# African-Robotics-Unit/AcinoSet

Hardware: AMD Instinct MI355X
Metric: FTE frames/sec (residual+Jac+LM step), 6-cam x 20-joint (higher is better)
Workload: dtype f64

## Files before the change

acinoset_amd/_lib.py:

```python
import ctypes as C
import os
import subprocess

_HERE = os.path.dirname(os.path.abspath(__file__))
_CSRC = os.path.join(_HERE, "csrc")
SO_PATH = os.path.join(_HERE, "libacinoset_hip.so")
BUILD_ID_SOURCE = "camera_kernels.hip"
SOURCES = ["camera_kernels.hip", "fte_assemble.hip", "bcr.hip", "seplevel.hip", "chunk.hip", "fte_cov.hip", "fte_calib.hip", "fte_reproj.hip", "fte_api.hip", "sba.hip", "sba_cov.hip", "ekf.hip", "ekf_cov.hip", "skel_fte.hip", "skel_cov.hip", "skel_cov_rates.hip", "skel_sample.hip", "skel_calib.hip", "skel_reproj.hip"]
HEADERS = ["common.hpp", "fte_kernels.hpp", "bcr.hpp", "bcr_dev.hpp", "seplevel.hpp", "chunk.hpp", "fte_cov.hpp", "fte_cov_dev.hpp", "fte_calib.hpp", "fte_reproj.hpp", "trio80.hpp", "dense80.hpp", "cheetah_fk.hpp",
           "pinhole.hpp", "ekf_dev.hpp", "sba_dev.hpp", "sba_host.hpp", "skel_dev.hpp", "skel_host.hpp", "skel_factor.hpp", "fte_assemble_body.inc", "ekf_forward_body.inc", "skel_assemble_body.inc",
           os.path.join("..", "..", "include", "acinoset_hip.h")]

ABI_VERSION = 3
N_ACTIVE = 25
N_STATES = 45
N_MARKERS = 20
CAM_STRIDE = 24
PINHOLE_STRIDE = 32
BS = 80
SEP_DOUBLES = 2 * BS * BS + BS


class FteParams(C.Structure):
    _fields_ = [("n_frames", C.c_int32), ("n_cams", C.c_int32), ("n_global", C.c_int64), ("n_offset", C.c_int64),
# ... 160 lines not shown
    "acino_sba_solve_sharded": (_I, [C.POINTER(SbaParams), _P, _P, _P, _P, _P, _P, _P, _P, _Z, _P, _P, C.POINTER(SbaInfo),
                                     REDUCE_FN, _P, _P]),
    "acino_sizeof_sba_cov_info": (_Z, []),
    "acino_sba_covariance_workspace_bytes": (_Z, [_I, _L, _L]),
    "acino_sba_covariance": (_I, [C.POINTER(SbaParams), _P, _P, _P, _P, _P, _P, _P, _I, _I, _I, _P, _I, _P, _Z, _P, _P, _P,
                                  C.POINTER(SbaCovInfo), _P]),
    "acino_sizeof_ekf_params": (_Z, []),
    "acino_ekf_workspace_bytes": (_Z, [_L, _I]),
    "acino_ekf_run": (_I, [C.POINTER(EkfParams), _P, _P, _P, _P, _Z, _P, _P, _P, _P]),
    "acino_ekf_run_pinhole": (_I, [C.POINTER(EkfParams), _P, _P, _P, _P, _Z, _P, _P, _P, _P]),
    "acino_ekf_smoothed_covariance": (_I, [C.POINTER(EkfParams), _P, _Z, _P, _P]),
    "acino_ekf_marker_covariance": (_I, [C.POINTER(EkfParams), _P, _P, _P, _P, _P, _P]),
    "acino_skeleton_fk": (_I, [_P, _L, _I, _I, C.POINTER(SkelOp), _I, _P, _P]),
    "acino_sizeof_skel_fte_params": (_Z, []),
    "acino_sizeof_skel_fte_info": (_Z, []),
    "acino_skel_fte_workspace_bytes": (_Z, [C.POINTER(SkelFteParams)]),
    "acino_skel_fte_workspace_bytes_batch": (_Z, [C.POINTER(SkelFteParams), _I]),
    "acino_skel_fte_solve": (_I, [C.POINTER(SkelFteParams), C.POINTER(SkelOp), C.POINTER(C.c_int32), _P, _P, _P, _P, _P, _P, _P,
                                  _P, _Z, C.POINTER(SkelFteInfo), _P]),
    "acino_skel_fte_solve_batch": (_I, [C.POINTER(SkelFteParams), _I, C.POINTER(SkelOp), C.POINTER(C.c_int32), _P, _P, _P, _P, _P,
                                        _P, _P, _P, _Z, C.POINTER(SkelFteInfo), _P]),
    "acino_skel_fte_solve_pinhole": (_I, [C.POINTER(SkelFteParams), C.POINTER(SkelOp), C.POINTER(C.c_int32), _P, _P, _P, _P, _P, _P,
                                          _P, _P, _Z, C.POINTER(SkelFteInfo), _P]),
    "acino_skel_fte_solve_batch_pinhole": (_I, [C.POINTER(SkelFteParams), _I, C.POINTER(SkelOp), C.POINTER(C.c_int32), _P, _P, _P,
                                                _P, _P, _P, _P, _P, _Z, C.POINTER(SkelFteInfo), _P]),
    "acino_skel_fte_covariance_workspace_bytes": (_Z, [C.POINTER(SkelFteParams), _I]),
    "acino_skel_fte_covariance": (_I, [C.POINTER(SkelFteParams), _I, _I, C.POINTER(SkelOp), C.POINTER(C.c_int32), _P, _P, _P, _P, _P,
                                       _P, _P, _P, _P, C.POINTER(C.c_int32), _P, _Z, _P]),
    "acino_skel_fte_sample_workspace_bytes": (_Z, [C.POINTER(SkelFteParams), _I, _L]),
    "acino_skel_fte_sample": (_I, [C.POINTER(SkelFteParams), _I, _I, C.POINTER(SkelOp), C.POINTER(C.c_int32), _P, _P, _P, _P, _P,
                                   _P, _L, _P, _P, _P, C.POINTER(C.c_int32), _P, _Z, _P]),
    "acino_skel_fte_observability_workspace_bytes": (_Z, [C.POINTER(SkelFteParams), _I]),
    "acino_skel_fte_observability": (_I, [C.POINTER(SkelFteParams), _I, _I, C.POINTER(SkelOp), C.POINTER(C.c_int32), _P, _P, _P, _P,
                                          _P, _P, _P, _P, _P, _P, _Z, _P]),
    "acino_skel_fte_covariance_pinned_workspace_bytes": (_Z, [C.POINTER(SkelFteParams), _I, _I]),
    "acino_skel_fte_covariance_pinned": (_I, [C.POINTER(SkelFteParams), _I, _I, C.POINTER(SkelOp), C.POINTER(C.c_int32), _P, _P, _P,
                                              _P, _P, _P, _P, _P, _P, C.POINTER(C.c_int32), _P, _Z, _P, _I, _P]),
    "acino_skel_fte_covariance_rates_workspace_bytes": (_Z, [C.POINTER(SkelFteParams), _I, _I]),
    "acino_skel_fte_covariance_rates": (_I, [C.POINTER(SkelFteParams), _I, _I, C.POINTER(SkelOp), C.POINTER(C.c_int32), _P, _P, _P,
                                             _P, _P, _P, _P, _P, _P, _P, _P, _P, _P, C.POINTER(C.c_int32), _P, _Z, _P, _I, _P]),
    "acino_skel_fte_sample_pinned_workspace_bytes": (_Z, [C.POINTER(SkelFteParams), _I, _L, _I]),
    "acino_skel_fte_sample_pinned": (_I, [C.POINTER(SkelFteParams), _I, _I, C.POINTER(SkelOp), C.POINTER(C.c_int32), _P, _P, _P, _P,
                                          _P, _P, _L, _P, _P, _P, C.POINTER(C.c_int32), _P, _Z, _P, _I, _P]),
    "acino_skel_fte_calibration_workspace_bytes": (_Z, [C.POINTER(SkelFteParams), _I, _I]),
    "acino_skel_fte_calibration_sensitivity": (_I, [C.POINTER(SkelFteParams), _I, _I, C.POINTER(SkelOp), C.POINTER(C.c_int32), _P, _P,
                                                    _P, _P, _P, _P, _P, _P, _P, _P, _P, C.POINTER(C.c_int32), _P, _Z, _P, _I, _P]),
    "acino_skel_fte_reprojection": (_I, [C.POINTER(SkelFteParams), _I, _I, C.POINTER(SkelOp), C.POINTER(C.c_int32), _P, _P, _P, _P,
                                         _P, _D, _P, _P, _P, _P, _P, _P]),
    "acino_skel_fte_reprojection_weights": (_I, [C.POINTER(SkelFteParams), _I, _I, C.POINTER(SkelOp), C.POINTER(C.c_int32), _P, _P, _P,
                                                 _P, _P, _D, _P, _P, _P, _P, _P, _P, _P]),
    "acino_selftest_mfma": (_I, [_P, _P, _I, _P, _P]),
    "acino_debug_poison_lds": (_I, [_I, _I, _P]),
    "acino_debug_level_split": (_I, [_I, _P]),
}

_lib = None


def source_hash():
    import hashlib
    h = hashlib.sha256()
    for rel in sorted(SOURCES + HEADERS):
        path = os.path.join(_CSRC, rel)
        h.update(os.path.basename(rel).encode())
        with open(path, "rb") as f:
            h.update(f.read())
    return h.hexdigest()[:16]


def built_id():
    if not os.path.exists(SO_PATH):
        return None
    with open(SO_PATH, "rb") as f:
        blob = f.read()
    i = blob.find(b"ACINO_BUILD_ID=")
    if i < 0:
        return None
    return blob[i + 15:i + 31].decode("ascii", "replace")


def _needs_build():
    return built_id() != source_hash()


def build(force=False, verbose=False):
    if not force and not _needs_build():
        return SO_PATH
    import hashlib
    from concurrent.futures import ThreadPoolExecutor
    hipcc = os.environ.get("HIPCC", "/opt/rocm/bin/hipcc")
    if not os.path.exists(hipcc):
        hipcc = "hipcc"
    sid = source_hash()
    hdr = hashlib.sha256()
    for rel in sorted(HEADERS):
        with open(os.path.join(_CSRC, rel), "rb") as f:
            hdr.update(f.read())
    objdir = os.path.join(_CSRC, "_obj")
    os.makedirs(objdir, exist_ok=True)
    flags = ["--offload-arch=gfx950", "-O3", "-std=c++17", "-fPIC", "-DNDEBUG"]
    jobs = []
    for src in SOURCES:
        with open(os.path.join(_CSRC, src), "rb") as f:
            key = hashlib.sha256(hdr.digest() + f.read() + " ".join(flags).encode()).hexdigest()[:16]
        extra = [f'-DACINO_BUILD_ID="{sid}"'] if src == BUILD_ID_SOURCE else []
        if extra:
# ... 96 lines not shown
```

acinoset_amd/csrc/bcr_dev.hpp:

```cpp
#pragma once
#include "bcr.hpp"
#include "dense80.hpp"

namespace acino {

__device__ __forceinline__ int tri_i(int t) { return (t >= 1) + (t >= 3) + (t >= 6) + (t >= 10); }
__device__ __forceinline__ int tri_j(int t) {
  const int i = tri_i(t);
  return t - (i * (i + 1)) / 2;
}

constexpr int LOWER_ITEMS = 1920;
__device__ __forceinline__ void lower_item(int idx, int& row, int& col) {
  const int ib = (idx >= 128) + (idx >= 384) + (idx >= 768) + (idx >= 1280);
  const int rem = idx - 64 * ib * (ib + 1), w = 8 * (ib + 1);
  row = 16 * ib + rem / w;
  col = 2 * (rem % w);
}

struct NodeFetch {
  double hv[8];
  double xv, gv, lam;
  bool row_live;
};
// ... 88 lines not shown
  return build_finish(Dm, bv, f, K, t, tid, K.q_w, K.lo, K.hi);
}

template <int NTH = 256>
static __device__ void publish_gmax(double gmax, double* red, double* gn_part, int node, int tid) {
  for (int off = 32; off > 0; off >>= 1) gmax = fmax(gmax, __shfl_down(gmax, off, 64));
  if ((tid & 63) == 0) red[tid >> 6] = gmax;
  __syncthreads();
  if (tid == 0) {
    double v = red[0];
#pragma unroll
    for (int w = 1; w < NTH / 64; ++w) v = fmax(v, red[w]);
    gn_part[node] = v;
  }
}

template <int NTH, class QW>
static __device__ __forceinline__ void fill_coupling_coef_q(double* coefL, double* coefR, const FteConst& K, int node_i,
                                                            int tid, QW qw) {
  const int loc_i = 3 * (node_i - K.pin_left);
  const int64_t f_i = K.n_offset + (int64_t)loc_i;
  for (int e = tid; e < 2 * 9 * NP; e += NTH) {
    const int side = e / (9 * NP), q = e % (9 * NP), pair = q / NP, p = q % NP, ii = pair / 3, jj = pair % 3;
    if (side == 0 ? !coefL : !coefR) continue;
    double v = 0.0;
    if (ii <= jj) {
      const int k = 3 + ii - jj;
      const int hi = side == 0 ? loc_i + ii : loc_i + 3 + ii;
      if (hi < K.n_frames)
        v = 2.0 * qw(p) * (side == 0 ? band_coef_clip(f_i - 3 + jj, k, K.n_global, K.clip_len)
                                             : band_coef_clip(f_i + jj, k, K.n_global, K.clip_len));
    }
    if (side == 0) coefL[q] = v;
    else coefR[q] = v;
  }
}
template <int NTH = 256>
static __device__ __forceinline__ void fill_coupling_coef(double* coefL, double* coefR, const FteConst& K, int node_i, int tid) {
  fill_coupling_coef_q<NTH>(coefL, coefR, K, node_i, tid, [&](int p) { return K.q_w[p]; });
}
template <int NTH = 256>
static __device__ __forceinline__ void fill_coupling_coef(double* coefL, double* coefR, const FteConst& K, int node_i, int tid,
                                                          const double* qw) {
  fill_coupling_coef_q<NTH>(coefL, coefR, K, node_i, tid, [&](int p) { return qw[p]; });
}

static __device__ __forceinline__ bool coupling_tables_uniform(const FteConst& K, int first, int last) {
  if (K.clip_len > 0) return false;
  const int64_t lo = K.n_offset + 3 * (int64_t)(first - K.pin_left) - 3;
  const int64_t hi = K.n_offset + 3 * (int64_t)(last - K.pin_left) + 5;
  return lo >= 3 && hi + 3 <= K.n_global - 4 && 3 * (last - K.pin_left) + 5 < K.n_frames;
}

static __device__ __forceinline__ bool right_table_is_interior(const FteConst& K, int node) {
  const int loc = 3 * (node - K.pin_left);
  const int64_t f = K.n_offset + (int64_t)loc;
  const int64_t len = K.clip_len > 0 ? K.clip_len : K.n_global;
  const int64_t r = K.clip_len > 0 ? f % K.clip_len : f;
  return f >= 0 && r <= len - 6 && f + 5 < K.n_global && loc + 5 < K.n_frames;
}
template <int NTH, class QW>
static __device__ __forceinline__ void right_table_interior(double* coefR, int tid, QW qw) {
  for (int q = tid; q < 9 * NP; q += NTH) {
    const int pair = q / NP, p = q % NP, ii = pair / 3, jj = pair % 3;
    coefR[q] = ii <= jj ? 2.0 * qw(p) * (jj == ii ? -1.0 : (jj - ii == 1 ? 6.0 : -15.0)) : 0.0;
  }
}

__device__ __forceinline__ double* ybuf(const BcrChain& ch) { return ch.Y ? ch.Y : ch.b; }

template <int NTH>
__device__ __forceinline__ void load_node_sum(double* Lm, double* yv, const BcrChain& ch, int i, int fl, int tid) {
  constexpr int NQ = (LOWER_ITEMS + NTH - 1) / NTH;
  const size_t MB = (size_t)BS * BS;
  const double* Dg = ch.D + i * MB;
  const bool hal = ch.AL0 != nullptr, hsl = (fl & 1) != 0, hsr = (fl & 2) != 0;
  const double* Ag = hal ? ch.AL0 + i * MB : Dg;
  const double* Lg = hsl ? ch.SL + i * MB : Dg;
  const double* Rg = hsr ? ch.SR + i * MB : Dg;
  double2 dv[NQ], av[NQ], lv[NQ], rv[NQ];
#pragma unroll
  for (int k = 0; k < NQ; ++k) {
    const int idx = tid + NTH * k;
    if (idx < LOWER_ITEMS) {
      int rr, cc;
      lower_item(idx, rr, cc);
      dv[k] = *reinterpret_cast<const double2*>(Dg + rr * BS + cc);
      av[k] = *reinterpret_cast<const double2*>(Ag + rr * BS + cc);
      lv[k] = *reinterpret_cast<const double2*>(Lg + rr * BS + cc);
      rv[k] = *reinterpret_cast<const double2*>(Rg + rr * BS + cc);
    }
  }
  double bb = 0.0, ab = 0.0, lb = 0.0, rb = 0.0;
  if (tid < BS) {
    bb = ch.b[(size_t)i * BS + tid];
    const int c = tid < 3 * NP ? tid : 0;
    ab = Ag[(size_t)(BS - 1) * BS + c];
    lb = Lg[(size_t)(BS - 1) * BS + c];
    rb = Rg[(size_t)(BS - 1) * BS + c];
  }
#pragma unroll
  for (int k = 0; k < NQ; ++k) {
    const int idx = tid + NTH * k;
    if (idx < LOWER_ITEMS) {
      int rr, cc;
      lower_item(idx, rr, cc);
      const bool in0 = rr < 3 * NP && cc < 3 * NP, in1 = rr < 3 * NP && cc + 1 < 3 * NP;
      double x = dv[k].x, y = dv[k].y;
      x += (hal && in0) ? av[k].x : 0.0;
      y += (hal && in1) ? av[k].y : 0.0;
      x += (hsl && in0) ? lv[k].x : 0.0;
      y += (hsl && in1) ? lv[k].y : 0.0;
// ... 19 lines not shown
```

acinoset_amd/csrc/chunk.hip:

```cpp
#include "chunk.hpp"

#include <algorithm>
#include <cstdlib>
#include <type_traits>

#include "bcr_dev.hpp"
#include "trio80.hpp"

namespace acino {

void ChunkPlan::build(int nodes_total, int chunk_nodes, bool pin_l, bool pin_r) {
  n_nodes = nodes_total;
  m = n_chunks = n_sep = 0;
  node0 = pin_l ? 1 : 0;
  pin_right = pin_r ? 1 : 0;
  const int nodes = nodes_total - node0;
  if (chunk_nodes < 0 || nodes < 1) return;
  int mm = chunk_nodes;
  if (mm == 0) {
    mm = (nodes + 255) / 256;
    mm = std::max(4, std::min(mm, 512));
  }
  mm = std::max(2, mm);
  m = mm;
// ... 119 lines not shown
__device__ __forceinline__ void gram_fetch(const double* X, int li, int lk, double (&a)[GramTile<T>::ns], double (&b)[GramTile<T>::ns]) {
  const double* pa = X + (GramTile<T>::ib * 16 + li) * LD + GramTile<T>::ib * 16 + lk;
  const double* pb = X + (GramTile<T>::jb * 16 + li) * LD + GramTile<T>::ib * 16 + lk;
#pragma unroll
  for (int s = 0; s < GramTile<T>::ns; ++s) {
    a[s] = pa[4 * s];
    b[s] = pb[4 * s];
  }
}
template <int T>
__device__ __forceinline__ void gram_tile(double* Xg, int li, int lk, const double (&a)[GramTile<T>::ns], const double (&b)[GramTile<T>::ns]) {
  constexpr int ib = GramTile<T>::ib, jb = GramTile<T>::jb;
  d4 g = {0, 0, 0, 0};
#pragma unroll
  for (int s = 0; s < GramTile<T>::ns; ++s) g = mfma(a[s], b[s], g);
#pragma unroll
  for (int rr = 0; rr < 4; ++rr) {
    Xg[(ib * 16 + lk + 4 * rr) * LD + jb * 16 + li] = g[rr];
    if (ib != jb) Xg[(jb * 16 + li) * LD + ib * 16 + lk + 4 * rr] = g[rr];
  }
}
template <int T0, int... REST>
__device__ __forceinline__ void gram_chain(const double* Xf, double* Xg, int li, int lk, const double (&a)[GramTile<T0>::ns],
                                           const double (&b)[GramTile<T0>::ns]) {
  if constexpr (sizeof...(REST) > 0) {
    constexpr int rest[] = {REST...};
    double an[GramTile<rest[0]>::ns], bn[GramTile<rest[0]>::ns];
    gram_fetch<rest[0]>(Xf, li, lk, an, bn);
    __builtin_amdgcn_sched_barrier(0);
    gram_tile<T0>(Xg, li, lk, a, b);
    __builtin_amdgcn_sched_barrier(0);
    gram_chain<REST...>(Xf, Xg, li, lk, an, bn);
  } else {
    gram_tile<T0>(Xg, li, lk, a, b);
  }
}
template <int T0, int... REST>
__device__ __forceinline__ void gram_fixed(const double* Xf, double* Xg, int* done, int li, int lk, int lane) {
  double a[GramTile<T0>::ns], b[GramTile<T0>::ns];
  gram_fetch<T0>(Xf, li, lk, a, b);
  gram_chain<T0, REST...>(Xf, Xg, li, lk, a, b);
  asm volatile("" ::: "memory");
  if (lane == 0) __hip_atomic_fetch_add(done, 1 + (int)sizeof...(REST), __ATOMIC_RELAXED, __HIP_MEMORY_SCOPE_WORKGROUP);
  asm volatile("" ::: "memory");
}

struct SpikeArgs {
  const double* Xg;
  double* Y;
  double* Ag;
  const double* cRk;
  const double* bvn;
  double* zk;
  int *c_gfdone, *c_fready, *c_bv, *tdone;
  int *g_open, *g_done;
  const double* Xf;
  int k, n_s;
  bool hasL, has_next;
  long long* stamps;
};
template <int ROLE>
__device__ __forceinline__ void spike_node(const SpikeArgs& A, int& tsb, int ln) {
  constexpr bool two = ROLE == 5;
  constexpr int j0 = ROLE == 4 ? 1 : (ROLE == 5 ? 2 : (ROLE == 6 ? 3 : 4));
  constexpr int NA = ROLE == 4 ? 3 : (ROLE == 5 ? 2 : (ROLE == 6 ? 5 : 4));
  const int li = ln & 15, lk = ln >> 4;
  double* const Y = A.Y;
  auto stamp = [&](int i) { if (A.stamps && ln == 0) A.stamps[i] = (long long)wall_clock64(); };
  AlTiles<NA> al;
  AlTiles<1> al0;
  al.Ag = A.Ag;
  al.j = j0;
  if (ROLE == 4) { al.as[0] = 1; al.as[1] = 0; al.as[2 % NA] = 2; }
  if (ROLE == 5) { al.as[0] = 2; al.as[1] = 0; }
  if (ROLE == 6) { al.as[0] = 3; al.as[1] = 0; al.as[2 % NA] = 1; al.as[3 % NA] = 2; al.as[4 % NA] = 4; }
  if (ROLE == 7) { al.as[0] = 4; al.as[1] = 0; al.as[2 % NA] = 1; al.as[3 % NA] = 2; }
  al0.Ag = A.Ag;
  al0.j = 0;
  al0.as[0] = 0;
  if (A.hasL) {
    al.fetch(li, lk);
    if (two) al0.fetch(li, lk);
  }
  if (ROLE >= 6) {
    double* const Xg = const_cast<double*>(A.Xg);
    lds_wait(A.g_open, A.k + 1);
    if (ROLE == 6) gram_fixed<2, 13>(A.Xf, Xg, A.g_done, li, lk, ln);
    else if (A.hasL) gram_fixed<5, 9, 14>(A.Xf, Xg, A.g_done, li, lk, ln);
    else gram_fixed<2, 5, 9, 13, 14>(A.Xf, Xg, A.g_done, li, lk, ln);
  }
  lds_wait(A.g_done, 15 * (A.k + 1));
  stamp(16 + 4 * (ROLE - 4));
  d4 T0[NT], T1[NT];
  {
    double bF[NT][4];
    const double* yb = Y + lk * LD + j0 * 16 + li;
#pragma unroll
    for (int kb = 0; kb < NT; ++kb)
#pragma unroll
      for (int s = 0; s < 4; ++s) bF[kb][s] = (4 * kb + s < SP_STEPS) ? yb[(kb * 16 + 4 * s) * LD] : 0.0;
    spike_gf(A.Xg, bF, T0, li, lk);
  }
  if (two) {
    double bF[NT][4];
    const double* yb = Y + lk * LD + li;
#pragma unroll
// ... 18 lines not shown
  }
  (void)tsb;
#pragma unroll
  for (int ib = 0; ib < NT; ++ib) tile_store(Y, ib, j0, T0[ib], li, lk);
  if (two) {
#pragma unroll
    for (int ib = 0; ib < NT; ++ib) tile_store(Y, ib, 0, T1[ib], li, lk);
  }
  if (ROLE == 7) {
    A.zk[ln] = Y[ln * LD + (BS - 1)];
    if (ln < 16) A.zk[64 + ln] = Y[(64 + ln) * LD + (BS - 1)];
  }
  if (A.has_next) {
    lds_wait(A.c_bv, A.k + 1);
    const double* const cRk = A.cRk;
    const double* const bvn = A.bvn;
    const int p = ln % NP, cg = ln / NP;
#pragma unroll
    for (int h = 0; h < (two ? 2 : 1); ++h) {
      const int c_lo = 16 * (h ? 0 : j0);
      if (cg < 2) {
        const double e00 = cRk[(0 * 3 + 0) * NP + p], e01 = cRk[(0 * 3 + 1) * NP + p], e02 = cRk[(0 * 3 + 2) * NP + p];
        const double e11 = cRk[(1 * 3 + 1) * NP + p], e12 = cRk[(1 * 3 + 2) * NP + p], e22 = cRk[(2 * 3 + 2) * NP + p];
        const double b0 = bvn[p], b1 = bvn[NP + p], b2 = bvn[2 * NP + p];
        double fv[8][3];
#pragma unroll
        for (int q = 0; q < 8; ++q) {
          const int cc = c_lo + cg + 2 * q;
          fv[q][0] = Y[p * LD + cc];
          fv[q][1] = Y[(NP + p) * LD + cc];
          fv[q][2] = Y[(2 * NP + p) * LD + cc];
        }
#pragma unroll
        for (int q = 0; q < 8; ++q) {
          const int cc = c_lo + cg + 2 * q;
          const double f0 = fv[q][0], f1 = fv[q][1], f2 = fv[q][2];
          double o0 = -(e00 * f0 + e01 * f1 + e02 * f2), o1 = -(e11 * f1 + e12 * f2), o2 = -(e22 * f2);
          if (cc == BS - 1) {
            o0 += b0;
            o1 += b1;
            o2 += b2;
          }
          Y[p * LD + cc] = o0;
          Y[(NP + p) * LD + cc] = o1;
          Y[(2 * NP + p) * LD + cc] = o2;
        }
      }
      if (ln < 16)
        for (int r = 3 * NP; r < BS; ++r) Y[r * LD + c_lo + ln] = 0.0;
    }
  }
  lds_signal(A.c_fready, ln);
  stamp(19 + 4 * (ROLE - 4));
}


__global__ void __launch_bounds__(SW_T)
k_chunk_sweep(BcrChain ch, SepView sp, const FteConst* __restrict__ cst, int* numeric_err, const int* __restrict__ status,
                int m, int n_chunks, int node0, int pin_right) {
  extern __shared__ __attribute__((aligned(16))) char smem_raw[];
  if (status && *status != 0) return;
  double* const Xf = reinterpret_cast<double*>(smem_raw);
  double* const Xg = Xf + MAT;
  double* const Y = Xg + MAT;
  double* const cL = Y + MAT;
  double* const cR0 = cL + 9 * NP;
  double* const bvb = cR0 + 9 * NP;
  double* const red = bvb + 2 * BS;
  int* const sync = reinterpret_cast<int*>(red + 8);
  int* const cB = sync + 5;
  int* const tdone = sync + 2;
  int* const g_done = sync + 6;
  int* const g_open = sync + 10;
  int* const c_gfdone = sync + 7;
  int* const c_fready = sync + 8;
  int* const c_bv = sync + 9;
  double* const kq = red + 16;
  double* const klo = kq + NP;
  double* const khi = klo + NP;
  long long* const lst = reinterpret_cast<long long*>(khi + NP);
  const int tid = threadIdx.x, wave = tid >> 6, lane = tid & 63;
  const FteConst& K = *cst;
  const int c = blockIdx.x;
  const int first = node0 + c * m;
  const bool hasL = c > 0 || node0 > 0, hasR = c + 1 < n_chunks || pin_right;
  const int len = c + 1 < n_chunks ? m : ch.n_nodes - first;
  const int n_int = hasR ? len - 1 : len;
  const int sL = c - 1 + node0, sR = c + node0;
  const size_t MB = (size_t)BS * BS;
  const int role = __builtin_amdgcn_readfirstlane(role8(wave));
  const bool uni_tables = coupling_tables_uniform(K, first, first + n_int - 1);
  const int n_s = hasL ? 4 : 1;
  const bool builder = role <= 3;
  const bool strips = role >= 4 && (hasL || role == 7);
  double gmax_run = 0.0;
  long long* const dbgp = (ch.dbg && (long long)blockIdx.x == ch.dbg[64] && ch.dbg[66] == 0) ? ch.dbg : nullptr;
  const int dbg_k = dbgp ? (int)ch.dbg[65] : -1;
  if (dbgp && lane == 0) {
    const unsigned hw = __builtin_amdgcn_s_getreg((31 << 11) | 4);
    atomicOr(reinterpret_cast<unsigned long long*>(ch.dbg + 67), (unsigned long long)((hw >> 4) & 3) << (4 * wave));
    if (wave == 0) ch.dbg[68] = hw;
  }
#define SW_STAMP(i) do { if (dbgp && k == dbg_k && lane == 0) lst[i] = (long long)wall_clock64(); } while (0)
  if (tid < 16) sync[tid] = 0;
  if (tid < 64) lst[tid] = 0;
  if (dbgp && tid == 0) dbgp[70] = (long long)wall_clock64();
  if (c == 0 && node0) {
    for (int e = tid; e < BS * BS; e += SW_T) sp.D[e] = 0.0;
    if (tid < BS) sp.b[tid] = 0.0;
  }
  if (tid < NP) {
    kq[tid] = K.q_w[tid];
    klo[tid] = K.lo[tid];
    khi[tid] = K.hi[tid];
  }
  __syncthreads();

  TrioSync tsy;
  {
    NodeFetch f;
    build_fetch<SW_T>(f, ch, K, first, tid);
    fill_coupling_coef<SW_T>(cL, cR0, K, first, tid, kq);
    for (int e = tid; e < MAT; e += SW_T) Y[e] = 0.0;
    gmax_run = build_finish<SW_T>(Xf, bvb, f, K, first, tid, kq, klo, khi);
    __syncthreads();
    if (dbgp && tid == 0) lst[60] = (long long)wall_clock64();
    if (hasL)
      for (int e = tid; e < 9 * NP; e += SW_T) {
        const int pair = e / NP, p = e % NP, ii = pair / 3, jj = pair % 3;
        if (ii <= jj) Y[(ii * NP + p) * LD + jj * NP + p] = cL[e];
      }
    if (tid < BS) Y[tid * LD + (BS - 1)] = bvb[tid];
    __syncthreads();
    if (role < 3) chol80_trio(Xf, role, lane, numeric_err, sync, tsy);
    __syncthreads();
    if (dbgp && tid == 0) lst[61] = (long long)wall_clock64();
  }

  unsigned slot0 = 0, slot1 = 0;
  if (builder) {
    auto pack = [](int e, bool own, bool dg) {
      const int pa = e / 13, dd = e % 13, pc = pa + dd >= NP ? pa + dd - NP : pa + dd;
      return (unsigned)pa | (unsigned)pc << 5 | (unsigned)own << 10 | (unsigned)dg << 11 | (unsigned)(pa * LD + pc) << 12 | (unsigned)e << 23;
    };
    auto offdiag = [](int n) { return 13 * (n / 12) + 1 + n % 12; };
    const bool dg0 = role == 1 && lane < NP;
    const int n0 = role == 1 ? 192 + lane - NP : (role == 0 ? 0 : (role == 2 ? 64 : 128)) + lane;
    slot0 = pack(dg0 ? 13 * lane : offdiag(n0), true, dg0);
    const bool own1 = (role == 3 && lane < 35) || (role == 2 && lane < 34);
    slot1 = pack(own1 ? offdiag((role == 3 ? 231 : 266) + lane) : 0, own1, false);
  }
  int tb = 0, tsb = 0;
#pragma unroll 1
  for (int k = 0; k < n_int; ++k) {
    const int node = first + k, next = node + 1;
    const bool last = k + 1 == n_int;
    const bool has_next = !last || hasR;
    const int ln = opaque(lane);
    const int li = ln & 15, lk = ln >> 4;
    double* const cRk = (uni_tables || !(k & 1)) ? cR0 : cL;
    if (builder) {
      const int bw = role;
      const int bt = bw * 64 + ln;
      const int fb_next = 3 * (next - node0);
      const BuildSlot s0 = BuildSlot::unpack(opaque_u(slot0)), s1 = BuildSlot::unpack(opaque_u(slot1));
      const bool two = bw >= 2;
      double hq[2][3] = {{0, 0, 0}, {0, 0, 0}}, xq[3] = {0, 0, 0}, gq[3] = {0, 0, 0}, cvq[3] = {0, 0, 0}, lamq = 0.0;
      bool liveq[3] = {false, false, false}, ownq[3] = {false, false, false};
      if (has_next) {
        const int cur = ch.st->cur;
        const double* Hg = cur ? ch.H1 : ch.H0;
        lamq = ch.st->lam;
#pragma unroll
        for (int j = 0; j < 3; ++j)
          if (fb_next + j < K.n_frames) {
            hq[0][j] = Hg[(size_t)(fb_next + j) * HPAIRS + s0.e];
            if (two && s1.own) hq[1][j] = Hg[(size_t)(fb_next + j) * HPAIRS + s1.e];
          }
        if (s0.dg) {
          const int pdg = s0.pr;
          const double* xg = cur ? ch.x1 : ch.x0;
          const double* gg = cur ? ch.g1 : ch.g0;
#pragma unroll
          for (int j = 0; j < 3; ++j)
            if (fb_next + j < K.n_frames) {
              xq[j] = xg[(size_t)(fb_next + j + HALO) * NP + pdg];
              gq[j] = gg[(size_t)(fb_next + j) * NP + pdg];
            }
#pragma unroll
          for (int pr = 0; pr < 3; ++pr) {
            const int j = pr == 2 ? 1 : 0, jp = pr == 0 ? 1 : 2;
            if (fb_next + jp < K.n_frames)
              cvq[pr] = 2.0 * kq[pdg] * band_coef_clip(K.n_offset + fb_next + j, jp - j, K.n_global, K.clip_len);
          }
        }
#pragma unroll
        for (int j = 0; j < 3; ++j) {
          liveq[j] = fb_next + j < K.n_frames;
          ownq[j] = fb_next + j >= K.own_lo && fb_next + j < K.own_hi;
        }
      }
      if (bw == 0) SW_STAMP(0);
      lds_barrier(cB, tb, 4, ln);
      lds_wait(c_gfdone, n_s * k);
      if (bw == 0) SW_STAMP(1);
      if (bt == 0) __hip_atomic_fetch_add(g_open, 1, __ATOMIC_RELAXED, __HIP_MEMORY_SCOPE_WORKGROUP);
      if (k > 0 && !uni_tables) fill_coupling_coef<256>(nullptr, cRk, K, node, bt, kq);
      if (bw == 0) gram_fixed<0, 10>(Xf, Xg, g_done, li, lk, ln);
      else if (bw == 1) gram_fixed<1, 7>(Xf, Xg, g_done, li, lk, ln);
      else if (bw == 2) gram_fixed<4, 8, 12>(Xf, Xg, g_done, li, lk, ln);
      else gram_fixed<3, 6, 11>(Xf, Xg, g_done, li, lk, ln);
      SW_STAMP(32 + wave);
      lds_barrier(cB, tb, 4, ln);
      lds_wait(g_done, 15 * (k + 1));
      if (bw == 0) SW_STAMP(2);
#pragma unroll
      for (int j = 0; j < 3; ++j) asm volatile("" : "+v"(hq[0][j]), "+v"(hq[1][j]), "+v"(xq[j]), "+v"(gq[j]));
      asm volatile("" : "+v"(lamq));
      if (has_next) {
        double* const bvn = bvb + ((k + 1) & 1) * BS;
        double ca[2][6], cb[2][6], gv[2][3][3];
        auto slot_reads = [&](const BuildSlot& sl, double (&a)[6], double (&b)[6], double (&g)[3][3]) {
          const double *ta = cRk + sl.pr, *tb_ = cRk + sl.pc;
          a[0] = ta[0 * NP]; a[1] = ta[1 * NP]; a[2] = ta[2 * NP];
          a[3] = ta[4 * NP]; a[4] = ta[5 * NP]; a[5] = ta[8 * NP];
          b[0] = tb_[0 * NP]; b[1] = tb_[1 * NP]; b[2] = tb_[2 * NP];
          b[3] = tb_[4 * NP]; b[4] = tb_[5 * NP]; b[5] = tb_[8 * NP];
          const double* gp0 = Xg + sl.base;
#pragma unroll
          for (int jj = 0; jj < 3; ++jj) {
            const double* gp = gp0 + jj * NP * LD;
            g[jj][0] = gp[0];
            g[jj][1] = gp[NP];
            g[jj][2] = gp[2 * NP];
          }
        };
        auto slot_finish = [&](const BuildSlot& sl, auto may_diag, const double (&a)[6], const double (&b)[6], const double (&g)[3][3],
                               const double (&h)[3]) {
#pragma clang fp contract(off)
          constexpr bool DIAG = decltype(may_diag)::value;
          const int pr = sl.pr;
          const bool dg = DIAG && sl.dg;
          const double a00 = a[0], a01 = a[1], a02 = a[2], a11 = a[3], a12 = a[4], a22 = a[5];
          const double b00 = b[0], b01 = b[1], b02 = b[2], b11 = b[3], b12 = b[4], b22 = b[5];
          double mm[3][3], S[2][3];
#pragma unroll
          for (int jj = 0; jj < 3; ++jj) {
            const double g0 = g[jj][0], g1 = g[jj][1], g2 = g[jj][2];
            mm[jj][0] = __builtin_fma(g2, b02, __builtin_fma(g0, b00, g1 * b01));
            mm[jj][1] = __builtin_fma(g1, b11, g2 * b12);
            mm[jj][2] = g2 * b22;
          }
#pragma unroll
          for (int ii = 0; ii < 3; ++ii) {
            S[0][ii] = __builtin_fma(a02, mm[2][ii], __builtin_fma(a00, mm[0][ii], a01 * mm[1][ii]));
            S[1][ii] = __builtin_fma(a11, mm[1][ii], a12 * mm[2][ii]);
          }
          double v[3][3];
#pragma unroll
          for (int j = 0; j < 3; ++j)
// ... 6 lines not shown
              if (liveq[j]) {
                d = h[j];
                const double gtol = GRAD_ZERO_REL * d;
                const bool fixed = (xq[j] <= klo[pr] && gq[j] > gtol) || (xq[j] >= khi[pr] && gq[j] < -gtol);
                d = __builtin_fma(lamq, fmax(d, DIAG_FLOOR), d);
                if (fixed) d *= FIX_SCALE;
                bb = fixed ? 0.0 : -gq[j];
                if (ownq[j]) gmax_run = fmax(gmax_run, fabs(bb));
              }
              v[j][j] = d;
              bvn[j * NP + pr] = bb;
            }
            v[0][1] = v[1][0] = cvq[0];
            v[0][2] = v[2][0] = cvq[1];
            v[1][2] = v[2][1] = cvq[2];
          }
          double val[3][3];
#pragma unroll
          for (int jp = 0; jp < 3; ++jp) {
            val[0][jp] = v[0][jp] - S[0][jp];
            val[1][jp] = v[1][jp] - S[1][jp];
          }
          val[2][0] = __builtin_fma(-a22, mm[2][0], v[2][0]);
          val[2][1] = v[2][1] - a22 * mm[2][1];
          val[2][2] = __builtin_fma(-a22, mm[2][2], v[2][2]);
          if (sl.own) {
            double* const xa = Xf + sl.base;
            double* const xt = Xf + sl.pc * LD + pr;
#pragma unroll
            for (int j = 0; j < 3; ++j)
#pragma unroll
              for (int jp = 0; jp < 3; ++jp) {
                xa[j * NP * LD + jp * NP] = val[j][jp];
                if (!dg) xt[jp * NP * LD + j * NP] = val[j][jp];
              }
          }
        };
        const BuildSlot b0 = BuildSlot::unpack(opaque_u(slot0)), b1 = BuildSlot::unpack(opaque_u(slot1));
        slot_reads(b0, ca[0], cb[0], gv[0]);
        slot_finish(b0, std::true_type{}, ca[0], cb[0], gv[0], hq[0]);
        if (two) {
          slot_reads(b1, ca[1], cb[1], gv[1]);
          slot_finish(b1, std::false_type{}, ca[1], cb[1], gv[1], hq[1]);
        }
        if (bt < BS - 3 * NP) {
          Xf[(3 * NP + bt) * LD + 3 * NP + bt] = 1.0;
          bvn[3 * NP + bt] = 0.0;
        }
      }
      lds_barrier(cB, tb, 4, ln);
      if (bt == 0) __hip_atomic_fetch_add(c_bv, 1, __ATOMIC_RELAXED, __HIP_MEMORY_SCOPE_WORKGROUP);
      if (bw == 0) SW_STAMP(4);
      if (bw < 3) {
        if (!last) chol80_trio<false>(Xf, bw, ln, numeric_err, sync, tsy, (dbgp && k == dbg_k) ? lst : nullptr);
        SW_STAMP(8 + wave);
      } else if (bw == 3) {
        double* Gg = ch.D + node * MB;
#pragma unroll 6
        for (int q = 0; q < LOWER_ITEMS / 64; ++q) {
          const int idx = ln + 64 * q;
          int r, cc;
          lower_item(idx, r, cc);
          *reinterpret_cast<double2*>(Gg + r * BS + cc) = make_double2(Xg[r * LD + cc], Xg[r * LD + cc + 1]);
        }
        SW_STAMP(8 + wave);
      }
    }
    if (strips) {
      SpikeArgs sa;
      sa.Xg = Xg; sa.Y = Y; sa.Ag = sp.AL + (size_t)(hasL ? opaque(sL) : 0) * MB; sa.cRk = cRk; sa.bvn = bvb + ((k + 1) & 1) * BS;
      sa.zk = ch.b + (size_t)node * BS; sa.g_open = g_open; sa.g_done = g_done; sa.Xf = Xf; sa.c_gfdone = c_gfdone; sa.c_fready = c_fready; sa.c_bv = c_bv; sa.tdone = tdone;
      sa.k = k; sa.n_s = n_s; sa.hasL = hasL; sa.has_next = has_next; sa.stamps = (dbgp && k == dbg_k) ? lst : nullptr;
      if (role == 4) spike_node<4>(sa, tsb, ln);
      else if (role == 5) spike_node<5>(sa, tsb, ln);
      else if (role == 6) spike_node<6>(sa, tsb, ln);
      else spike_node<7>(sa, tsb, ln);
    }
  }
  __syncthreads();
  if (dbgp) {
    if (tid == 0) lst[62] = (long long)wall_clock64();
    __syncthreads();
    if (tid < 64 && lst[tid]) dbgp[tid] = lst[tid];
  }
  if (hasR) {
    {
      double2* d2 = reinterpret_cast<double2*>(sp.D + (size_t)sR * MB);
      for (int idx = tid; idx < BS * BS / 2; idx += SW_T) {
        const int e = 2 * idx, r = e / BS, cc = e % BS;
        d2[idx] = make_double2(Xf[r * LD + cc], Xf[r * LD + cc + 1]);
      }
    }
    if (tid < BS) sp.b[(size_t)sR * BS + tid] = Y[tid * LD + (BS - 1)];
    if (hasL) {
      double* Cg = sp.Cpl + (size_t)sL * MB;
      for (int e = tid; e < BS * BS; e += SW_T) {
        const int r = e / BS, cc = e % BS;
        Cg[e] = cc < 3 * NP ? Y[r * LD + cc] : 0.0;
      }
    }
  }
#undef SW_STAMP
  publish_gmax<SW_T>(gmax_run, red, ch.gn_part, c, tid);
  if (dbgp && tid == 0) dbgp[71] = (long long)wall_clock64();
}

__global__ void __launch_bounds__(256) k_sep_combine(SepView sp, const int* __restrict__ status) {
  if (status && *status != 0) return;
  const int q = blockIdx.x, tid = threadIdx.x;
  const size_t MB = (size_t)BS * BS;
  double* D = sp.D + q * MB;
  const double* A = sp.AL + q * MB;
  constexpr int NQ = (LOWER_ITEMS + 255) / 256;
  double2 dv[NQ], av[NQ];
  const double bq = tid < 3 * NP ? sp.b[(size_t)q * BS + tid] : 0.0, aq = tid < 3 * NP ? A[(size_t)(BS - 1) * BS + tid] : 0.0;
#pragma unroll
  for (int k = 0; k < NQ; ++k) {
    const int idx = tid + 256 * k;
    if (idx < LOWER_ITEMS) {
      int r, cc;
      lower_item(idx, r, cc);
      dv[k] = *reinterpret_cast<const double2*>(D + r * BS + cc);
      av[k] = *reinterpret_cast<const double2*>(A + r * BS + cc);
    }
  }
#pragma unroll
  for (int k = 0; k < NQ; ++k) {
    const int idx = tid + 256 * k;
    if (idx < LOWER_ITEMS) {
      int r, cc;
      lower_item(idx, r, cc);
      if (r < 3 * NP) {
        const double ax = cc < 3 * NP ? av[k].x : 0.0, ay = cc + 1 < 3 * NP ? av[k].y : 0.0;
        *reinterpret_cast<double2*>(D + r * BS + cc) = make_double2(dv[k].x + ax, dv[k].y + ay);
      }
    }
  }
  if (tid < 3 * NP) sp.b[(size_t)q * BS + tid] = bq + aq;
}

constexpr int BK_PW = 4;
constexpr int BK_NL = 4;
constexpr int BK_T = 64 * (BK_PW + BK_NL);
constexpr int BK_NB = 2;
constexpr int BLD = 82;
constexpr int BK_Q = LOWER_ITEMS / 64;
constexpr int BK_FL = 8;
static_assert(LOWER_ITEMS == 64 * NT * (NT + 1), "30 rounds of 64 items: 2 (ib + 1) per tile row");
static_assert(BK_FL >= BK_NL + BK_NB + 2, "a far f_k must have been stored (and waited for) before a loader asks for it");
constexpr int BK_OPS = BS * BLD, BK_TAB = BK_OPS + 5 * BS, BK_STAGE = BK_TAB + 9 * NP + 1;
static constexpr size_t kBacksubLds =
    (BK_NB * BK_STAGE + 2 * BS + BK_FL * BS + 2 * 9 * NP + 16 + NP + 1) * sizeof(double) + 16 * sizeof(int);

// ... 312 lines not shown
      sp_ += red[2 * w];
      sm = fmax(sm, red[2 * w + 1]);
    }
    trial.pred_part[c] = sp_;
    trial.step_part[c] = sm;
  }
}

int chunk_set_func_attributes() {
  ACINO_HIP_CHECK(hipFuncSetAttribute(reinterpret_cast<const void*>(k_chunk_sweep),
                                      hipFuncAttributeMaxDynamicSharedMemorySize, (int)kSweepLds));
  ACINO_HIP_CHECK(hipFuncSetAttribute(reinterpret_cast<const void*>(k_chunk_backsub),
                                      hipFuncAttributeMaxDynamicSharedMemorySize, (int)kBacksubLds));
  return ACINO_OK;
}

int chunk_reduce(const BcrChain& ch, const ChunkPlan& pl, const SepView& sp, const BcrChain& sepch,
                 const BcrSchedule& sepsch, const FteConst* d_c, int* d_numeric_err, const int* d_status, hipStream_t s,
                 Profiler* prof) {
  {
    ProfSpan span(prof, PC_CHUNK_SWEEP, s, pl.n_nodes - pl.n_sep);
    hipLaunchKernelGGL(k_chunk_sweep, dim3(pl.n_chunks), dim3(SW_T), kSweepLds, s, ch, sp, d_c, d_numeric_err, d_status, pl.m,
                       pl.n_chunks, pl.node0, pl.pin_right);
  }
  ACINO_LAUNCH_CHECK();
  if (pl.n_sep == 0) return ACINO_OK;
  if (!sepsch.consumers_add_al) {
    {
      ProfSpan span(prof, PC_SEP_COMBINE, s, pl.n_sep);
      hipLaunchKernelGGL(k_sep_combine, dim3(pl.n_sep), dim3(256), 0, s, sp, d_status);
    }
    ACINO_LAUNCH_CHECK();
  }
  return bcr_reduce(sepch, sepsch, d_c, d_numeric_err, d_status, s, prof);
}

int chunk_backsub(const BcrChain& ch, const ChunkPlan& pl, const SepView& sp, const BcrChain& sepch,
                  const BcrSchedule& sepsch, const FteConst* d_c, int* d_numeric_err, const int* d_status, hipStream_t s,
                  Profiler* prof, const TrialOut& trial) {
  if (pl.n_sep > 0) {
    int rc = bcr_backsub(sepch, sepsch, d_c, d_status, s, prof, d_numeric_err);
    if (rc) return rc;
  }
  {
    ProfSpan span(prof, PC_CHUNK_BACKSUB, s, pl.n_nodes - pl.n_sep);
    hipLaunchKernelGGL(k_chunk_backsub, dim3(pl.n_chunks), dim3(BK_T), kBacksubLds, s, ch, sp, d_c, d_status, pl.m, pl.n_chunks, pl.node0,
                       pl.pin_right, trial);
  }
  ACINO_LAUNCH_CHECK();
  return ACINO_OK;
}

}
```

include/acinoset_hip.h:

```cpp
#ifndef ACINOSET_HIP_H
#define ACINOSET_HIP_H

#include <stddef.h>
#include <stdint.h>

#ifdef __cplusplus
extern "C" {
#endif

#define ACINO_ABI_VERSION 3

typedef enum acino_status {
  ACINO_OK = 0,
  ACINO_ERR_INVALID_ARG = -1,
  ACINO_ERR_HIP = -2,
  ACINO_ERR_WORKSPACE = -3,
  ACINO_ERR_NO_DEVICE = -4,
  ACINO_ERR_UNSUPPORTED = -5,
  ACINO_ERR_NUMERIC = -6,
  ACINO_ERR_CALLBACK = -7
} acino_status;

#define ACINO_CAM_STRIDE 24
#define ACINO_PINHOLE_STRIDE 32
// ... 296 lines not shown

size_t acino_skel_fte_calibration_workspace_bytes(const acino_skel_fte_params* p, int n_clips, int pin_unobserved);
int acino_skel_fte_calibration_sensitivity(const acino_skel_fte_params* p, int n_clips, int camera_model, const acino_skel_op* h_ops,
                                           const int32_t* h_active, const double* d_meas, const double* d_w, const double* d_cams,
                                           const double* d_lo, const double* d_hi, const double* d_x,
                                           const double* d_cov_cams , double* d_sens, double* d_cov_x_cal,
                                           double* d_cov_pos_cal, double* d_std_pos_cal,
                                           int32_t* h_status , void* d_ws, size_t ws_bytes,
                                           void* stream, int pin_unobserved,
                                           uint8_t* d_unobserved );

int acino_skel_fte_reprojection(const acino_skel_fte_params* p, int n_clips, int camera_model ,
                                const acino_skel_op* h_ops, const int32_t* h_active, const double* d_meas, const double* d_w,
                                const double* d_cams, const double* d_x,
                                const double* d_cov_pos , double gate_w, double* d_uv,
                                double* d_cov_uv, double* d_res, double* d_mahal2, uint8_t* d_flags, void* stream);
int acino_skel_fte_reprojection_weights(const acino_skel_fte_params* p, int n_clips, int camera_model, const acino_skel_op* h_ops,
                                        const int32_t* h_active, const double* d_meas, const double* d_w, const double* d_cams,
                                        const double* d_x, const double* d_cov_pos, double gate_w, double* d_uv, double* d_cov_uv,
                                        double* d_res, double* d_mahal2, uint8_t* d_flags, double* d_weight, void* stream);

typedef struct acino_ekf_params {
  int64_t n_frames;
  int32_t n_seq;
  int32_t n_cams;
  double fps;
  double dlc_thresh;
  double cam_width;
  int32_t smoother_pivoting;
  int32_t reserved;
} acino_ekf_params;
size_t acino_sizeof_ekf_params(void);
size_t acino_ekf_workspace_bytes(int64_t n_frames, int n_seq);
int acino_ekf_run(const acino_ekf_params* prm, const double* d_det, const double* d_cams24, const double* d_states0,
                  void* d_ws, size_t ws_bytes, double* d_est, double* d_smooth, int32_t* d_outliers, void* stream);
int acino_ekf_run_pinhole(const acino_ekf_params* prm, const double* d_det, const double* d_cams32, const double* d_states0,
                          void* d_ws, size_t ws_bytes, double* d_est, double* d_smooth, int32_t* d_outliers, void* stream);
int acino_ekf_smoothed_covariance(const acino_ekf_params* prm, const void* d_ws, size_t ws_bytes, double* d_P_smooth,
                                  void* stream);
int acino_ekf_marker_covariance(const acino_ekf_params* prm, const double* d_states, const double* d_P, double* d_cov_pos,
                                double* d_std_pos, double* d_std_state, void* stream);

int acino_fte_graphs_active(acino_fte_ctx* ctx);
int acino_fte_shard_reduce(acino_fte_ctx* ctx, double* d_sep, int rank, int world, void* stream);
int acino_fte_shard_solve(acino_fte_ctx* ctx, const double* d_sep, double* d_sep_x, void* d_scratch, size_t scratch_bytes,
                          double* d_edge_out, int rank, int world, void* stream);
int acino_fte_shard_eval(acino_fte_ctx* ctx, int which, const double* d_all_edges, int rank, int world,
                         double* d_partial_out, void* stream);
int acino_fte_shard_control(acino_fte_ctx* ctx, const double* d_all_partials, int world, int init, void* stream);

int acino_debug_poison_lds(int n_blocks, int spin, void* stream);
int acino_selftest_mfma(const double* d_a, const double* d_b, int k, double* d_c, void* stream);
int acino_debug_level_split(int T, int32_t* out);

#ifdef __cplusplus
}
#endif
#endif
```

Baseline: 24.55 million.

## Fold separator epilogue stores into last chunk step and cache coupling tables

Replaces the uniform-table check with per-node tracking of two coupling-coefficient buffers, so the tables are only rewritten when a node's table changes, and interior tables use a cheap closed-form fill. The post-loop epilogue that copied the factor, right-hand side and coupling block to the separator arrays is moved into the last iteration, where idle Cholesky and spike waves do the work alongside other roles. This is meant to remove redundant table fills and a serialized tail phase. It adds more branching and extra LDS waits, and the table-tracking logic is easy to get wrong. A host debug entry point for checking table values is also added.

```diff
diff --git a/acinoset_amd/_lib.py b/acinoset_amd/_lib.py
--- a/acinoset_amd/_lib.py
+++ b/acinoset_amd/_lib.py
@@ -236,6 +236,7 @@
     "acino_selftest_mfma": (_I, [_P, _P, _I, _P, _P]),
     "acino_debug_poison_lds": (_I, [_I, _I, _P]),
     "acino_debug_level_split": (_I, [_I, _P]),
+    "acino_debug_coupling_table": (_I, [_L, _L, _L, _L, _I, _I, _P, _P]),
 }
 
 _lib = None
diff --git a/acinoset_amd/csrc/bcr_dev.hpp b/acinoset_amd/csrc/bcr_dev.hpp
--- a/acinoset_amd/csrc/bcr_dev.hpp
+++ b/acinoset_amd/csrc/bcr_dev.hpp
@@ -164,12 +164,30 @@
   return lo >= 3 && hi + 3 <= K.n_global - 4 && 3 * (last - K.pin_left) + 5 < K.n_frames;
 }
 
-static __device__ __forceinline__ bool right_table_is_interior(const FteConst& K, int node) {
-  const int loc = 3 * (node - K.pin_left);
-  const int64_t f = K.n_offset + (int64_t)loc;
-  const int64_t len = K.clip_len > 0 ? K.clip_len : K.n_global;
-  const int64_t r = K.clip_len > 0 ? f % K.clip_len : f;
-  return f >= 0 && r <= len - 6 && f + 5 < K.n_global && loc + 5 < K.n_frames;
+struct TableGeom {
+  int64_t n_global, n_offset, clip_len;
+  int32_t n_frames, pin_left;
+};
+static __host__ __device__ __forceinline__ TableGeom table_geom(const FteConst& K) {
+  return TableGeom{K.n_global, K.n_offset, K.clip_len, K.n_frames, K.pin_left};
+}
+static __host__ __device__ __forceinline__ bool right_table_is_interior(const TableGeom& G, int node) {
+  const int loc = 3 * (node - G.pin_left);
+  const int64_t f = G.n_offset + (int64_t)loc;
+  const int64_t len = G.clip_len > 0 ? G.clip_len : G.n_global;
+  const int64_t r = G.clip_len > 0 ? f % G.clip_len : f;
+  return f >= 0 && r <= len - 6 && f + 5 < G.n_global && loc + 5 < G.n_frames;
+}
+static __host__ __device__ __forceinline__ bool right_table_is_interior(const FteConst& K, int node) {
+  return right_table_is_interior(table_geom(K), node);
+}
+static __host__ __device__ __forceinline__ bool left_table_is_interior(const TableGeom& G, int node) {
+  return right_table_is_interior(G, node - 1);
+}
+static __host__ __device__ __forceinline__ double right_table_band(const TableGeom& G, int node, int ii, int jj) {
+  const int loc = 3 * (node - G.pin_left);
+  if (ii > jj || loc + 3 + ii >= G.n_frames) return 0.0;
+  return band_coef_clip(G.n_offset + (int64_t)loc + jj, 3 + ii - jj, G.n_global, G.clip_len);
 }
 template <int NTH, class QW>
 static __device__ __forceinline__ void right_table_interior(double* coefR, int tid, QW qw) {
diff --git a/acinoset_amd/csrc/chunk.hip b/acinoset_amd/csrc/chunk.hip
--- a/acinoset_amd/csrc/chunk.hip
+++ b/acinoset_amd/csrc/chunk.hip
@@ -195,6 +195,7 @@
   const double* cRk;
   const double* bvn;
   double* zk;
+  double *Cg, *bR;
   int *c_gfdone, *c_fready, *c_bv, *tdone;
   int *g_open, *g_done;
   const double* Xf;
@@ -319,6 +320,17 @@
   }
   lds_signal(A.c_fready, ln);
   stamp(19 + 4 * (ROLE - 4));
+  if (A.bR) {
+    if (A.Cg && !two) {
+      const int cc = 16 * j0 + li;
+#pragma unroll 5
+      for (int r = lk; r < BS; r += 4) A.Cg[r * BS + cc] = cc < 3 * NP ? Y[r * LD + cc] : 0.0;
+    }
+    if (ROLE == 7) {
+      A.bR[ln] = Y[ln * LD + (BS - 1)];
+      if (ln < 16) A.bR[64 + ln] = Y[(64 + ln) * LD + (BS - 1)];
+    }
+  }
 }
 
 
@@ -356,7 +368,10 @@
   const int sL = c - 1 + node0, sR = c + node0;
   const size_t MB = (size_t)BS * BS;
   const int role = __builtin_amdgcn_readfirstlane(role8(wave));
-  const bool uni_tables = coupling_tables_uniform(K, first, first + n_int - 1);
+  const TableGeom TG = table_geom(K);
+  const bool left_int = left_table_is_interior(TG, first);
+  int tab_cur = 0;
+  bool tab_int0 = right_table_is_interior(TG, first), tab_int1 = left_int;
   const int n_s = hasL ? 4 : 1;
   const bool builder = role <= 3;
   const bool strips = role >= 4 && (hasL || role == 7);
@@ -387,7 +402,14 @@
   {
     NodeFetch f;
     build_fetch<SW_T>(f, ch, K, first, tid);
-    fill_coupling_coef<SW_T>(cL, cR0, K, first, tid, kq);
+    if (left_int && tab_int0) {
+      if (tid < 2 * 9 * NP) {
+        const int q = tid % (9 * NP), pair = q / NP, p = q % NP, ii = pair / 3, jj = pair % 3;
+        cL[tid] = ii <= jj ? 2.0 * kq[p] * (jj == ii ? -1.0 : (jj - ii == 1 ? 6.0 : -15.0)) : 0.0;
+      }
+    } else {
+      fill_coupling_coef<SW_T>(cL, cR0, K, first, tid, kq);
+    }
     for (int e = tid; e < MAT; e += SW_T) Y[e] = 0.0;
     gmax_run = build_finish<SW_T>(Xf, bvb, f, K, first, tid, kq, klo, khi);
     __syncthreads();
@@ -425,7 +447,17 @@
     const bool has_next = !last || hasR;
     const int ln = opaque(lane);
     const int li = ln & 15, lk = ln >> 4;
-    double* const cRk = (uni_tables || !(k & 1)) ? cR0 : cL;
+    bool tab_write = false, tab_interior = false;
+    if (k > 0) {
+      tab_interior = right_table_is_interior(TG, node);
+      if (!(tab_interior && (tab_cur ? tab_int1 : tab_int0))) {
+        tab_cur ^= 1;
+        tab_write = !(tab_interior && (tab_cur ? tab_int1 : tab_int0));
+        if (tab_cur) tab_int1 = tab_interior;
+        else tab_int0 = tab_interior;
+      }
+    }
+    double* const cRk = tab_cur ? cL : cR0;
     if (builder) {
       const int bw = role;
       const int bt = bw * 64 + ln;
@@ -472,7 +504,10 @@
       lds_wait(c_gfdone, n_s * k);
       if (bw == 0) SW_STAMP(1);
       if (bt == 0) __hip_atomic_fetch_add(g_open, 1, __ATOMIC_RELAXED, __HIP_MEMORY_SCOPE_WORKGROUP);
-      if (k > 0 && !uni_tables) fill_coupling_coef<256>(nullptr, cRk, K, node, bt, kq);
+      if (tab_write) {
+        if (tab_interior) right_table_interior<256>(cRk, bt, [&](int p) { return kq[p]; });
+        else fill_coupling_coef<256>(nullptr, cRk, K, node, bt, kq);
+      }
       if (bw == 0) gram_fixed<0, 10>(Xf, Xg, g_done, li, lk, ln);
       else if (bw == 1) gram_fixed<1, 7>(Xf, Xg, g_done, li, lk, ln);
       else if (bw == 2) gram_fixed<4, 8, 12>(Xf, Xg, g_done, li, lk, ln);
@@ -585,7 +620,24 @@
       if (bt == 0) __hip_atomic_fetch_add(c_bv, 1, __ATOMIC_RELAXED, __HIP_MEMORY_SCOPE_WORKGROUP);
       if (bw == 0) SW_STAMP(4);
       if (bw < 3) {
-        if (!last) chol80_trio<false>(Xf, bw, ln, numeric_err, sync, tsy, (dbgp && k == dbg_k) ? lst : nullptr);
+        if (!last) {
+          chol80_trio<false>(Xf, bw, ln, numeric_err, sync, tsy, (dbgp && k == dbg_k) ? lst : nullptr);
+        } else if (hasR) {
+          double2* d2 = reinterpret_cast<double2*>(sp.D + (size_t)sR * MB);
+          for (int idx = bt; idx < BS * BS / 2; idx += 192) {
+            const int e = 2 * idx, r = e / BS, cc = e % BS;
+            d2[idx] = make_double2(Xf[r * LD + cc], Xf[r * LD + cc + 1]);
+          }
+          if (hasL) {
+            double* const Cg = sp.Cpl + (size_t)sL * MB;
+            lds_wait(c_fready, n_s * (k + 1));
+#pragma unroll 7
+            for (int idx = bt; idx < 2 * BS * 8; idx += 192) {
+              const int h = idx / (BS * 8), rem = idx % (BS * 8), r = rem >> 3, cc = (h ? 32 : 0) + 2 * (rem & 7);
+              *reinterpret_cast<double2*>(Cg + r * BS + cc) = make_double2(Y[r * LD + cc], Y[r * LD + cc + 1]);
+            }
+          }
+        }
         SW_STAMP(8 + wave);
       } else if (bw == 3) {
         double* Gg = ch.D + node * MB;
@@ -603,6 +655,8 @@
       SpikeArgs sa;
       sa.Xg = Xg; sa.Y = Y; sa.Ag = sp.AL + (size_t)(hasL ? opaque(sL) : 0) * MB; sa.cRk = cRk; sa.bvn = bvb + ((k + 1) & 1) * BS;
       sa.zk = ch.b + (size_t)node * BS; sa.g_open = g_open; sa.g_done = g_done; sa.Xf = Xf; sa.c_gfdone = c_gfdone; sa.c_fready = c_fready; sa.c_bv = c_bv; sa.tdone = tdone;
+      sa.bR = (last && hasR) ? sp.b + (size_t)sR * BS : nullptr;
+      sa.Cg = (last && hasR && hasL) ? sp.Cpl + (size_t)sL * MB : nullptr;
       sa.k = k; sa.n_s = n_s; sa.hasL = hasL; sa.has_next = has_next; sa.stamps = (dbgp && k == dbg_k) ? lst : nullptr;
       if (role == 4) spike_node<4>(sa, tsb, ln);
       else if (role == 5) spike_node<5>(sa, tsb, ln);
@@ -615,23 +669,6 @@
     if (tid == 0) lst[62] = (long long)wall_clock64();
     __syncthreads();
     if (tid < 64 && lst[tid]) dbgp[tid] = lst[tid];
-  }
-  if (hasR) {
-    {
-      double2* d2 = reinterpret_cast<double2*>(sp.D + (size_t)sR * MB);
-      for (int idx = tid; idx < BS * BS / 2; idx += SW_T) {
-        const int e = 2 * idx, r = e / BS, cc = e % BS;
-        d2[idx] = make_double2(Xf[r * LD + cc], Xf[r * LD + cc + 1]);
-      }
-    }
-    if (tid < BS) sp.b[(size_t)sR * BS + tid] = Y[tid * LD + (BS - 1)];
-    if (hasL) {
-      double* Cg = sp.Cpl + (size_t)sL * MB;
-      for (int e = tid; e < BS * BS; e += SW_T) {
-        const int r = e / BS, cc = e % BS;
-        Cg[e] = cc < 3 * NP ? Y[r * LD + cc] : 0.0;
-      }
-    }
   }
 #undef SW_STAMP
   publish_gmax<SW_T>(gmax_run, red, ch.gn_part, c, tid);
@@ -1050,3 +1087,17 @@
 }
 
 }
+
+extern "C" int acino_debug_coupling_table(int64_t n_global, int64_t n_frames, int64_t n_offset, int64_t clip_len, int pin_left,
+                                          int node, int32_t* interior, double* coef) {
+  using namespace acino;
+  ACINO_REQUIRE(interior && coef, "outputs");
+  ACINO_REQUIRE(n_global >= 1 && n_frames >= 1 && n_frames <= INT32_MAX && n_offset >= 0 && n_offset + n_frames <= n_global &&
+                    clip_len >= 0 && (pin_left == 0 || pin_left == 1),
+                "a window of n_frames frames at n_offset inside n_global frames");
+  const TableGeom G{n_global, n_offset, clip_len, (int32_t)n_frames, pin_left};
+  *interior = right_table_is_interior(G, node) ? 1 : 0;
+  for (int ii = 0; ii < 3; ++ii)
+    for (int jj = 0; jj < 3; ++jj) coef[3 * ii + jj] = right_table_band(G, node, ii, jj);
+  return ACINO_OK;
+}
diff --git a/include/acinoset_hip.h b/include/acinoset_hip.h
--- a/include/acinoset_hip.h
+++ b/include/acinoset_hip.h
@@ -372,6 +372,8 @@
 int acino_debug_poison_lds(int n_blocks, int spin, void* stream);
 int acino_selftest_mfma(const double* d_a, const double* d_b, int k, double* d_c, void* stream);
 int acino_debug_level_split(int T, int32_t* out);
+int acino_debug_coupling_table(int64_t n_global, int64_t n_frames, int64_t n_offset, int64_t clip_len, int pin_left, int node,
+                               int32_t* interior, double* coef);
 
 #ifdef __cplusplus
 }
```

Result: faster. 24.95 million (median of 6 runs) (+1.6%).
